# hyeeiin/ECG-Multimodal-Model

Hardware: AMD Instinct MI355X
Metric: samples/sec fwd+bwd, batch-256 multimodal (img+sig+clin), 1->8 MI355X (higher is better)
Workload: dtype bf16; 1 GPU; full multimodal (image 3x224x224 + 5000-pt signal + 16-dim clinical), fwd+bwd+Adam, encoders unfrozen; image_hw=224x224, per_gpu_batch=256, global_batch=256, parallelism=dp1

## Files before the change

ecg-multimodal-model_amd/csrc/api.hip:

```cpp
#include <stdarg.h>

#include "ops.h"

static thread_local char g_err[512] = "";

void ecg_set_error(const char* fmt, ...) {
  va_list ap;
  va_start(ap, fmt);
  vsnprintf(g_err, sizeof(g_err), fmt, ap);
  va_end(ap);
}

static inline ConvGeom geom_of(const ecgmm_conv_desc* c) {
  return make_geom(c->N, c->H, c->W, c->Cin, c->Cout, c->R, c->S, c->stride, c->pad_h, c->pad_w);
}
#define S_(x) ((hipStream_t)(x))

extern "C" {

int ecgmm_version(void) { return ECGMM_VERSION; }
const char* ecgmm_last_error(void) { return g_err; }

const char* ecgmm_switch_name(int i) { return i >= 0 && i < sw::COUNT ? sw::ALL[i]->env : nullptr; }
int ecgmm_switch_get(const char* env_name, int64_t* value) {
// ... 3 lines not shown
  *value = s->get();
  return 0;
}
int ecgmm_switch_set(const char* env_name, int64_t value) {
  Switch* s = sw::find(env_name);
  if (!s) ECG_FAIL(ECGMM_ERR_SHAPE, "switch_set: unknown switch %s", env_name ? env_name : "(null)");
  if (s == &sw::SIDE_WGRAD)
    ECG_FAIL(ECGMM_ERR_SHAPE, "switch_set: ECGMM_SIDE_WGRAD is each plan's own state after start-up, call ecgmm_side_wgrad()");
  if (!s->runtime) ECG_FAIL(ECGMM_ERR_SHAPE, "switch_set: %s is read once at start-up", s->env);
  s->set((long)value);
  return 0;
}
int ecgmm_conv_halo_enable(int on) { sw::CONV_HALO.set(on); return 0; }
int ecgmm_conv_halo_cus(int cus) { sw::HALO_CUS.set(cus); return 0; }
int ecgmm_conv_halo_w4(int on) { sw::HALO_W4.set(on); return 0; }
int ecgmm_conv_halo_stagger(int on) { sw::HALO_STAGGER.set(on); return 0; }
int ecgmm_conv_halo_stream(int on) { sw::HALO_STREAM.set(on); return 0; }
int ecgmm_conv_halo_pingpong(int on) { sw::HALO_PP.set(on); return 0; }
int ecgmm_conv_wgrad_pingpong(int on) { sw::WGRAD_PP.set(on); return 0; }
int ecgmm_conv_wgrad_ring_enable(int on) { sw::WGRAD_RING.set(on); return 0; }
int ecgmm_bn_fold(int on) { sw::BN_FOLD.set(on); return 0; }
int ecgmm_bn_fold_slice(int on) { sw::BN_FOLD_SLICE.set(on); return 0; }
int ecgmm_bn_dual(int on) { ecg_bn_dual_set(on); return 0; }
int ecgmm_bn_fuse_min_pixels(int64_t m) { sw::BN_FUSE_MIN_M.set((long)m); return 0; }
int ecgmm_stem_recompute(int on) { sw::STEM_RECOMPUTE.set(on); return 0; }
int ecgmm_infer_down_side(int on) { sw::INFER_DOWN_SIDE.set(on); return 0; }

int ecgmm_nchw_to_nhwc(int dtype, const float* src, void* dst, int N, int C, int64_t HW, void* stream) {
  return ecg_nchw_to_nhwc(dtype, src, dst, N, C, (long)HW, S_(stream));
}
int ecgmm_nhwc_to_nchw(int dtype, const void* src, float* dst, int N, int C, int64_t HW, void* stream) {
  return ecg_nhwc_to_nchw(dtype, src, dst, N, C, (long)HW, S_(stream));
}
int ecgmm_cast(int dtype, const float* src, void* dst, int64_t n, void* stream) {
  return ecg_cast(dtype, src, dst, (long)n, S_(stream));
}
int ecgmm_uncast(int dtype, const void* src, float* dst, int64_t n, void* stream) {
  return ecg_uncast(dtype, src, dst, (long)n, S_(stream));
}
int ecgmm_pack_conv_weight(int dtype, const float* w, void* fwd, void* dgrad, int Cout, int Cin, int RS,
                           void* stream) {
  return ecg_pack_weight(dtype, w, fwd, dgrad, Cout, Cin, RS, S_(stream));
}

int ecgmm_conv_stats_rows(int64_t out_pixels) { return ecg_conv_stats_rows((long)out_pixels); }
int ecgmm_conv_fwd(int dtype, const ecgmm_conv_desc* c, const void* x, const void* w_fwd, const float* bias, void* y,
// ... 28 lines not shown
}
int ecgmm_stem_stats_only_rows(int N, int Cin, int H, int W, int R) { return ecg_stem_stats_only_rows(N, Cin, H, W, R); }
int ecgmm_stem_stats_only(int dtype, const float* x, const void* packed, const float* bias, float* stats, int N, int Cin,
                          int H, int W, int R, void* stream) {
  return ecg_stem_stats_only(dtype, x, packed, bias, stats, N, Cin, H, W, R, S_(stream));
}
int ecgmm_stem_pool_fwd(const float* x, const void* packed, const float* coef, void* pooled, uint8_t* idx, int N, int Cin,
                        int H, int W, void* stream) {
  return ecg_stem_pool_fwd(x, packed, coef, pooled, idx, N, Cin, H, W, S_(stream));
}
size_t ecgmm_stem_pool_bwd_workspace(int N, int Cin, int H, int W) { return ecg_stem_pool_bwd_workspace(N, Cin, H, W); }
int ecgmm_stem_pool_bwd(const float* x, const void* packed, const float* coef, const float* gamma, const void* dp,
                        const void* pooled, const uint8_t* idx, float* dgamma, float* dbeta, float* dw_oihw, void* ws,
                        size_t ws_bytes, int N, int Cin, int H, int W, void* stream) {
  return ecg_stem_pool_bwd(x, packed, coef, gamma, dp, pooled, idx, dgamma, dbeta, dw_oihw, ws, ws_bytes, N, Cin, H, W,
                           S_(stream));
}
size_t ecgmm_stem_bwd_weight_workspace(int N, int Cin, int H, int W, int R) {
  return ecg_stem_wgrad_workspace(N, Cin, H, W, R);
}
int ecgmm_stem_bwd_weight(int dtype, const float* x, const void* dy, float* dw, int accumulate, void* ws,
                          size_t ws_bytes, int N, int Cin, int H, int W, int R, void* stream) {
  return ecg_stem_wgrad(dtype, x, dy, dw, accumulate, ws, ws_bytes, N, Cin, H, W, R, S_(stream));
}

int ecgmm_stem_bwd_data(int dtype, const void* dy, const float* w_oihw, float* dx, int N, int Cin, int H, int W, int R,
                        void* stream) {
  return ecg_stem_dgrad(dtype, dy, w_oihw, dx, N, Cin, H, W, R, S_(stream));
}

int ecgmm_bn_eval_bwd(int dtype, const void* dout, const void* maskref, const float* gate, const float* addc,
                      int rows_per_sample, const void* y, const float* coef, float* dgamma, float* dbeta, void* dy,
                      void* dz_out, float* dbias, int64_t M, int C, float* scratch, void* stream) {
  return ecg_bn_eval_bwd(dtype, dout, maskref, gate, addc, rows_per_sample, y, coef, dgamma, dbeta, dy, dz_out, dbias,
                         (long)M, C, scratch, S_(stream));
}
int ecgmm_bn_small_eval_bwd(const float* x, const float* dy, const float* gamma, const float* save, float* dx,
                            float* dgamma, float* dbeta, int N, int C, int accumulate, void* stream) {
  return ecg_bn_small_eval_bwd(x, dy, gamma, save, dx, dgamma, dbeta, N, C, accumulate, S_(stream));
}

int ecgmm_col_stats_rows(int dtype, int64_t M, int C) { return ecg_bn_rows(dtype, (long)M, C); }
int ecgmm_col_stats(int dtype, const void* x, int64_t M, int C, float* partial, void* stream) {
  int rows = 0;
  return ecg_col_stats(dtype, x, (long)M, C, partial, &rows, S_(stream));
}
// ... 298 lines not shown
```

ecg-multimodal-model_amd/csrc/conv_stem.hip:

```cpp
#include "ops.h"

__device__ __host__ inline size_t align_up_dev(size_t a) { return (a + 15) & ~(size_t)15; }

#ifndef STEM_ABL
#define STEM_ABL 0
#endif

namespace {

constexpr int STEM_CO = 64;
constexpr int MAXG = 24;

struct StemParams {
  const float* x;
  const void* wpk;
  void* y;
  const float* bias;
  float* stats;
  float* slab;
  int N, Cin, H, W, OH, OW, R, pad_h;
  int TH, TW;
  int tiles_h, tiles_w;
  int NG;
};
// ... 278 lines not shown
  }
#endif
  }
  __syncthreads();
  }
  if (STATS_WG && p.stats) {
    float* srow = p.stats + ((size_t)blockIdx.x * 4 + wave) * 2 * STEM_CO;
#pragma unroll
    for (int a = 0; a < 4; ++a) {
      f32x4 r1, r2;
#pragma unroll
      for (int j = 0; j < 4; ++j) {
        r1[j] = row16_sum(ws1[a][j]);
        r2[j] = row16_sum(ws2[a][j]);
      }
      if (fr == 0) {
        *reinterpret_cast<f32x4*>(srow + a * 16 + fq * 4) = r1;
        *reinterpret_cast<f32x4*>(srow + STEM_CO + a * 16 + fq * 4) = r2;
      }
    }
  }
}

template <typename T, int R>
__global__ __launch_bounds__(256) void stem_wgrad_kernel(StemParams p) {
  extern __shared__ __attribute__((aligned(16))) unsigned char smem[];
  constexpr int DYS = sizeof(T) == 2 ? 144 : 320;
  constexpr int TH = StemDims<R>::TH, TW = StemDims<R>::TW, PH = StemDims<R>::PH, PWS = StemDims<R>::PWS;
  unsigned char* sDY = smem;
  float* patch = reinterpret_cast<float*>(smem + 128 * DYS);

  const int tid = threadIdx.x, lane = tid & 63, wave = tid >> 6;
  const int fr = lane & 15, fq = lane >> 4;
  const int NK = p.NG * 8;
  const int ktiles = (NK + 15) / 16;
  const int tpi = p.tiles_h * p.tiles_w;
  const int vb = stem_xcd_order();
  const int pos = vb % tpi, slot = vb / tpi, nslots = gridDim.x / tpi;
  const int th_i = pos / p.tiles_w, tw_i = pos - th_i * p.tiles_w;
  const int oh0 = th_i * TH, ow0 = tw_i * TW;

  f32x4 acc[4][3];
#pragma unroll
  for (int a = 0; a < 4; ++a)
#pragma unroll
    for (int b = 0; b < 3; ++b) acc[a][b] = (f32x4){0.f, 0.f, 0.f, 0.f};

  int koff[3];
#pragma unroll
  for (int b = 0; b < 3; ++b) {
    const int kidx = (wave + 4 * b) * 16 + fr;
    const bool kok = (wave + 4 * b) < ktiles && kidx < NK;
    const int kk = kok ? kidx : 0;
    const int G = kk >> 3, c = G / R;
    koff[b] = (c * PH + (G - c * R)) * PWS + (kk & 7);
  }

  const T* dy = (const T*)p.y;
  constexpr int CH = 64 * (int)sizeof(T) / 16;
  constexpr int NDY = 128 * CH / 256;
  float pre[StemDims<R>::NPRE];
  u32x4 pdy[NDY];
  unsigned poff[StemDims<R>::NPRE], dyoff[NDY];
  stem_patch_offsets<R>(p, oh0, ow0, poff);
#pragma unroll
  for (int k = 0; k < NDY; ++k) {
    const int i = tid + 256 * k;
    const int pix = i / CH, chunk = i % CH;
    const int oh = oh0 + pix / TW, ow = ow0 + pix % TW;
    dyoff[k] = ((oh < p.OH) & (ow < p.OW)) ? (unsigned)(((oh * p.OW + ow) * STEM_CO) * (int)sizeof(T) + chunk * 16) : 0xFFFFFFFFu;
  }
  auto fetch = [&](int n) {
    const size_t dimg = (size_t)p.OH * p.OW * STEM_CO;
    const __amdgpu_buffer_rsrc_t drs = __builtin_amdgcn_make_buffer_rsrc((void*)(dy + (size_t)n * dimg), 0,
                                                                          (int)(dimg * sizeof(T)), 0x00020000);
#pragma unroll
    for (int k = 0; k < NDY; ++k) {
#if defined(__HIP_DEVICE_COMPILE__)
      pdy[k] = __builtin_amdgcn_raw_buffer_load_b128(drs, (int)dyoff[k], 0, 0);
#endif
    }
    stem_fetch_image_patch<R>(p, poff, pre, n);
  };
  if (slot < p.N) fetch(slot);
  for (int n = slot; n < p.N; n += nslots) {
    __syncthreads();
#pragma unroll
    for (int k = 0; k < NDY; ++k) {
      const int i = tid + 256 * k;
      *reinterpret_cast<u32x4*>(sDY + (i / CH) * DYS + (i % CH) * 16) = pdy[k];
    }
    stem_store_slots<float, R>(patch, pre);
    __syncthreads();
    if (n + nslots < p.N) fetch(n + nslots);

    if constexpr (sizeof(T) == 2) {
      const int q = fr >> 2, pq = fr & 3;
      for (int st = 0; st < 4; ++st) {
        u32x4 fa[4];
#pragma unroll
        for (int a = 0; a < 4; ++a) {
          const unsigned char* a0 = sDY + (st * 32 + 8 * fq + q) * DYS + (a * 16 + 4 * pq) * 2;
          s16x4 lo = __builtin_amdgcn_ds_read_tr16_b64_v4i16(
              (__attribute__((address_space(3))) s16x4*)(const_cast<unsigned char*>(a0)));
          s16x4 hi = __builtin_amdgcn_ds_read_tr16_b64_v4i16(
              (__attribute__((address_space(3))) s16x4*)(const_cast<unsigned char*>(a0 + 4 * DYS)));
          uint2 l2 = __builtin_bit_cast(uint2, lo), h2 = __builtin_bit_cast(uint2, hi);
          fa[a] = (u32x4){l2.x, l2.y, h2.x, h2.y};
        }
        const int pix0 = st * 32 + 8 * fq;
        const int trow = pix0 / TW, tcol0 = pix0 % TW;
#pragma unroll
        for (int b = 0; b < 3; ++b) {
          float bv[8];
          const float* src = patch + koff[b] + trow * 2 * PWS + tcol0 * 2;
#pragma unroll
          for (int j = 0; j < 8; ++j) bv[j] = src[2 * j];
          u32x4 fb = pack16<bf16_t>(bv);
#pragma unroll
          for (int a = 0; a < 4; ++a)
            mfma_bf16_inplace(acc[a][b], fa[a], fb);
        }
      }
    } else {
      for (int st = 0; st < 32; ++st) {
        const int pix = st * 4 + fq;
        const int trow = pix / TW, tcol = pix % TW;
        float fa[4];
#pragma unroll
        for (int a = 0; a < 4; ++a) fa[a] = *reinterpret_cast<const float*>(sDY + pix * DYS + (a * 16 + fr) * 4);
#pragma unroll
        for (int b = 0; b < 3; ++b) {
          float fb = patch[koff[b] + trow * 2 * PWS + tcol * 2];
#pragma unroll
          for (int a = 0; a < 4; ++a) acc[a][b] = __builtin_amdgcn_mfma_f32_16x16x4f32(fa[a], fb, acc[a][b], 0, 0, 0);
        }
      }
    }
  }

  if (sizeof(T) == 2) mfma_drain();
#pragma unroll
  for (int b = 0; b < 3; ++b) {
    int kidx = (wave + 4 * b) * 16 + fr;
    if ((wave + 4 * b) >= ktiles || kidx >= NK) continue;
#pragma unroll
    for (int a = 0; a < 4; ++a)
#pragma unroll
      for (int j = 0; j < 4; ++j)
        p.slab[((size_t)blockIdx.x * STEM_CO + a * 16 + fq * 4 + j) * NK + kidx] = acc[a][b][j];
  }
}

__global__ __launch_bounds__(256) void stem_wgrad_reduce_kernel(const float* __restrict__ slab,
                                                                float* __restrict__ grad, int nsplit, int NG,
                                                                int accumulate) {
  __shared__ float sh[16][17];
  const int oi = threadIdx.x & 15, sl = threadIdx.x >> 4;
  const int i = blockIdx.x * 16 + oi;
  const int total = STEM_CO * NG * 7;
  const int NK = NG * 8;
  float acc = 0.f;
  if (i < total) {
    int s = i % 7;
    int t = i / 7;
    int G = t % NG, co = t / NG;
    const float* src = slab + (size_t)co * NK + G * 8 + s;
    const size_t stride = (size_t)STEM_CO * NK;
    int k = sl;
    for (; k + 48 < nsplit; k += 64) {
      const float a0 = src[(size_t)k * stride], a1 = src[(size_t)(k + 16) * stride];
      const float a2 = src[(size_t)(k + 32) * stride], a3 = src[(size_t)(k + 48) * stride];
      acc += a0;
      acc += a1;
// ... 184 lines not shown
  if (!workspace || workspace_bytes < need)
    ECG_FAIL(ECGMM_ERR_WORKSPACE, "stem wgrad: workspace %zu < %zu", workspace_bytes, need);
  StemParams p;
  fill_params(p, s, N, Cin, H, W, R);
  p.x = x; p.y = const_cast<void*>(dy); p.slab = (float*)workspace;
  size_t lds = 128 * (size_t)(dtype == ECGMM_BF16 ? 144 : 320) + stem_patch_buffer_bytes(R, sizeof(float));
  if (dtype != ECGMM_BF16 && dtype != ECGMM_F32) ECG_FAIL(ECGMM_ERR_DTYPE, "stem wgrad: bad dtype %d", dtype);
  ecg_prof_begin(ECG_PROF_STEM_WGRAD, 2.0 * (double)N * s.OH * s.OW * STEM_CO * Cin * R * 7,
                 4.0 * N * Cin * H * W + (double)dtype_size(dtype) * N * s.OH * s.OW * STEM_CO, stream);
  if (dtype == ECGMM_BF16) {
    if (R == 7) hipLaunchKernelGGL((stem_wgrad_kernel<bf16_t, 7>), dim3(grid), dim3(256), lds, stream, p);
    else hipLaunchKernelGGL((stem_wgrad_kernel<bf16_t, 1>), dim3(grid), dim3(256), lds, stream, p);
  } else {
    if (R == 7) hipLaunchKernelGGL((stem_wgrad_kernel<float, 7>), dim3(grid), dim3(256), lds, stream, p);
    else hipLaunchKernelGGL((stem_wgrad_kernel<float, 1>), dim3(grid), dim3(256), lds, stream, p);
  }
  ecg_prof_end(stream);
  ECG_CHECK_LAUNCH("stem_wgrad");
  hipLaunchKernelGGL(stem_wgrad_reduce_kernel, dim3(ceil_div(STEM_CO * s.NG * 7, 16)), dim3(256), 0, stream,
                     (const float*)workspace, grad, grid, s.NG, accumulate);
  ECG_CHECK_LAUNCH("stem_wgrad_reduce");
  return 0;
}
```

ecg-multimodal-model_amd/csrc/ops.h:

```cpp
#pragma once
#include "common.h"
#include "switches.h"

int ecg_conv_stats_rows(long M);
struct ConvEpi {
  const void* red_y;
  const void* red_mask;
  const float* red_coef;
  float* red_rows;
  int wg_rows;
  const void* src2;
  const void* wpk2;
  int src2_done;
  int stats_rows;
  int red_done;
  int red_rows_n;
};
int ecg_conv_igemm(int dtype, int mode, const ConvGeom& g, const void* src, const void* wpk, void* dst,
                   const float* bias, const void* addend, float* stats, int act, hipStream_t stream,
                   ConvEpi* epi = nullptr);
bool ecg_conv_halo_ok(int dtype, int mode, const ConvGeom& g);
int ecg_conv_halo_rows(int mode, const ConvGeom& g);
int ecg_conv_halo(int mode, const ConvGeom& g, const void* src, const void* wpk, void* dst, const float* bias,
                  const void* addend, float* stats, int act, ConvEpi* epi, hipStream_t stream);
size_t ecg_conv_wgrad_workspace(int dtype, const ConvGeom& g);
void ecg_conv_wgrad_narrow(bool narrow, int slots = 256);
int ecg_conv_wgrad(int dtype, const ConvGeom& g, const void* x, const void* dy, float* grad_oihw, int accumulate,
                   void* workspace, size_t workspace_bytes, hipStream_t stream);
size_t ecg_stem_packed_elems(int Cin, int R);
int ecg_stem_stats_rows(int N, int Cin, int H, int W, int R);
int ecg_stem_pack(int dtype, const float* w, void* out, int Cin, int R, hipStream_t stream);
int ecg_stem_fwd(int dtype, const float* x, const void* wpk, const float* bias, void* y, float* stats, int N, int Cin,
                 int H, int W, int R, hipStream_t stream);
size_t ecg_stem_wgrad_workspace(int N, int Cin, int H, int W, int R);
int ecg_stem_wgrad(int dtype, const float* x, const void* dy, float* grad, int accumulate, void* workspace,
                   size_t workspace_bytes, int N, int Cin, int H, int W, int R, hipStream_t stream);
int ecg_stem_stats_only_rows(int N, int Cin, int H, int W, int R);
int ecg_stem_wg_stats_rows(int N, int Cin, int H, int W, int R);
int ecg_stem_fwd_wgrows(int dtype, const float* x, const void* wpk, const float* bias, void* y, float* stats, int N, int Cin,
                        int H, int W, int R, hipStream_t stream);
int ecg_stem_stats_only(int dtype, const float* x, const void* wpk, const float* bias, float* stats, int N, int Cin, int H,
                        int W, int R, hipStream_t stream);
int ecg_stem_wgrad_reduce(const float* slab, float* grad, int rows, int NG, int accumulate, hipStream_t stream);
int ecg_stem_dgrad(int dtype, const void* dy, const float* w, float* dx, int N, int Cin, int H, int W, int R,
                   hipStream_t stream);
bool ecg_stem_fused_ok(int dtype, int Cin, int R);
int ecg_stem_pool_fwd(const float* x, const void* wpk, const float* coef, void* pooled, unsigned char* idx, int N, int Cin,
                      int H, int W, hipStream_t stream);
size_t ecg_stem_pool_bwd_workspace(int N, int Cin, int H, int W);
int ecg_stem_pool_bwd(const float* x, const void* wpk, const float* coef, const float* gamma, const void* dp, const void* pooled,
                      const unsigned char* idx, float* dgamma, float* dbeta, float* dw, void* ws, size_t ws_bytes, int N,
                      int Cin, int H, int W, hipStream_t stream);
int ecg_pool_bn_bwd_reduce(int dtype, const void* dp, const void* pooled, const float* coef, const float* gamma, float* dgamma,
                           float* dbeta, int N, int H, int W, int C, float* scratch, const float** bcoef_out,
                           hipStream_t stream);
int ecg_bn_rows(int dtype, long M, int C);
int ecg_bn_finalize(const float* partial, int rows, int C, double count, const float* gamma, const float* beta,
                    float* rm, float* rv, long long* nbt, float momentum, float eps, float* coef, hipStream_t stream);
int ecg_bn_eval_coef(int C, const float* gamma, const float* beta, const float* rm, const float* rv, float eps,
                     float* coef, hipStream_t stream);
int ecg_col_stats(int dtype, const void* x, long M, int C, float* partial, int* rows_out, hipStream_t stream);
struct EcgBnFold {
  const float* partial; int rows; double count;
  const float* gamma; const float* beta;
  float* rm; float* rv; long long* nbt;
  float momentum, eps;
// ... 201 lines not shown
```

ecg-multimodal-model_amd/csrc/plan_resnet18.hip:

```cpp
#include "plan_common.h"
#include "side_stream.h"

namespace {
bool stem_recompute(int dtype) {
  return sw::STEM_RECOMPUTE.get() && ecg_stem_fused_ok(dtype, 3, 7);
}
bool relu_bits_on() { return sw::RELU_BITS.get() != 0; }

int build(const ecgmm_resnet18_desc* d, Net18& r) {
  ECG_TRY(net18_static(d, r, "resnet18"));
  return net18_shape(r, "resnet18");
}

struct FwdWs {
  void* wstem;
  void* y0; float* coef0; void* p0; unsigned char* idx0;
  BlockWs b[8];
  float* pooled;
  float* stats;
  float* stats_d;
  size_t bytes;
};

void layout_fwd(const Net18& r, void* base, FwdWs& w, WsTable* views = nullptr) {
// ... 375 lines not shown
        if (!sw::DOWN_FOLD.get()) ed.src2 = nullptr;
        if (ed.src2) {
          ECG_TRY(ecg_conv_igemm(dt, 1, g1, dy1b, b.w1d, din, nullptr, nullptr, nullptr, 0, s, &ed));
        }
        if (!ed.src2_done) {
          ECG_TRY(ecg_conv_igemm(dt, 1, gd, dydb, b.wdd, q.dtmp, nullptr, nullptr, nullptr, 0, s));
          ECG_TRY(ecg_conv_igemm(dt, 1, g1, dy1b, b.w1d, din, nullptr, q.dtmp, nullptr, 0, s));
        }
      } else {
        ConvEpi eb = {};
        if (fuse_here && i > 0 && ecg_conv_halo_ok(dt, 1, g1)) {
          const BlockWs& pb = w.b[i - 1];
          eb.wg_rows = 1; eb.red_y = pb.y2; eb.red_mask = pb.out; eb.red_coef = pb.coef2; eb.red_rows = q.red2;
        }
        ECG_TRY(ecg_conv_igemm(dt, 1, g1, dy1b, b.w1d, din, nullptr, dzp, nullptr, 0, s, &eb));
      }
    } else if (st == 9) {
      const void* dp0 = q.X[8 & 1];
      if (stem_recompute(dt)) {
        ECG_TRY(ecg_stem_pool_bwd(image, w.wstem, w.coef0, P(params, 1), dp0, w.p0, w.idx0, G(grads, 1), G(grads, 2),
                                  G(grads, 0), q.stem_ws, q.stem_bytes, N, 3, r.d.H, r.d.W, s));
        continue;
      }
      if (train && ecg_stem_fuse_on()) {
        ECG_TRY(ecg_pool_bn_bwd(dt, dp0, w.p0, w.idx0, w.y0, w.coef0, P(params, 1), G(grads, 1), G(grads, 2), q.big1,
                                nullptr, N, r.H1, r.W1, 64, q.bn_scratch, s));
      } else {
        ECG_TRY(ecg_maxpool_relu_bwd(dt, dp0, w.p0, w.idx0, q.big0, N, r.H1, r.W1, 64, s));
        ECG_TRY(bn_bwd_mode(r.bn, q.big0, nullptr, nullptr, nullptr, 1, w.y0, w.coef0, P(params, 1), G(grads, 1), G(grads, 2),
                            q.big1, nullptr, nullptr, (long)N * r.H1 * r.W1, 64, q.bn_scratch, s));
      }
      if (G(grads, 0)) {
        ECG_TRY(ecg_stem_wgrad(dt, image, q.big1, G(grads, 0), 0, q.stem_ws, q.stem_bytes, N, 3, r.d.H, r.d.W, 7, s));
      }
      if (dimage) ECG_TRY(ecg_stem_dgrad(dt, q.big1, P(params, 0), dimage, N, 3, r.d.H, r.d.W, 7, s));
    } else {
      ECG_FAIL(ECGMM_ERR_SHAPE, "resnet18 bwd: stage %d out of range", st);
    }
  }
  if (stage_end == 10) ecg_tl_mark(210, s);
  if (side && !g_side.defer_join) {
    hipEvent_t e = side_next_ev();
    (void)hipEventRecord(e, g_side.s);
    (void)hipStreamWaitEvent(s, e, 0);
  }
  if (stage_end == 10) ecg_tl_mark(211, s);
// ... 36 lines not shown
```

ecg-multimodal-model_amd/hip/lib.py:

```python
import ctypes as C
import os

F32, BF16 = 0, 1
ACT_NONE, ACT_RELU, ACT_SIGMOID = 0, 1, 2
RESNET18_NPARAMS, RESNET18_NBUFFERS = 62, 60
RESNET1D_NPARAMS, RESNET1D_NBUFFERS = 52, 27

_PKG_DIR = os.path.dirname(os.path.dirname(os.path.abspath(__file__)))
LIB_PATH = os.environ.get("ECGMM_LIB") or os.path.join(_PKG_DIR, "libecgmm_hip.so")

vp, i32, i64, u64, f32, f64, sz = C.c_void_p, C.c_int, C.c_int64, C.c_uint64, C.c_float, C.c_double, C.c_size_t


class ConvDesc(C.Structure):
    _fields_ = [(n, i32) for n in ("N", "H", "W", "Cin", "Cout", "R", "S", "stride", "pad_h", "pad_w")]


class ResNet18Desc(C.Structure):
    _fields_ = [("N", i32), ("H", i32), ("W", i32), ("out_dim", i32), ("dtype", i32), ("training", i32),
                ("bn_momentum", f32), ("bn_eps", f32)]


class ResNet1DDesc(C.Structure):
    _fields_ = [("N", i32), ("cin", i32), ("L", i32), ("num_classes", i32), ("dtype", i32), ("training", i32),
# ... 60 lines not shown
    "ecgmm_nhwc_to_nchw": (i32, [i32, vp, vp, i32, i32, i64, vp]),
    "ecgmm_cast": (i32, [i32, vp, vp, i64, vp]),
    "ecgmm_uncast": (i32, [i32, vp, vp, i64, vp]),
    "ecgmm_pack_conv_weight": (i32, [i32, vp, vp, vp, i32, i32, i32, vp]),
    "ecgmm_conv_stats_rows": (i32, [i64]),
    "ecgmm_conv_fwd": (i32, [i32, P(ConvDesc), vp, vp, vp, vp, vp, i32, vp]),
    "ecgmm_conv_fwd_wgrows": (i32, [i32, P(ConvDesc), vp, vp, vp, vp, vp, vp, i32, vp]),
    "ecgmm_conv_bwd_data": (i32, [i32, P(ConvDesc), vp, vp, vp, vp, vp]),
    "ecgmm_conv_bwd_weight_workspace": (sz, [i32, P(ConvDesc)]),
    "ecgmm_conv_bwd_weight": (i32, [i32, P(ConvDesc), vp, vp, vp, i32, vp, sz, vp]),
    "ecgmm_stem_packed_elems": (sz, [i32, i32]),
    "ecgmm_stem_stats_rows": (i32, [i32, i32, i32, i32, i32]),
    "ecgmm_stem_pack": (i32, [i32, vp, vp, i32, i32, vp]),
    "ecgmm_stem_fwd": (i32, [i32, vp, vp, vp, vp, vp, i32, i32, i32, i32, i32, vp]),
    "ecgmm_stem_wg_stats_rows": (i32, [i32, i32, i32, i32, i32]),
    "ecgmm_stem_fwd_wgrows": (i32, [i32, vp, vp, vp, vp, vp, i32, i32, i32, i32, i32, vp]),
    "ecgmm_stem_stats_only_rows": (i32, [i32, i32, i32, i32, i32]),
    "ecgmm_stem_stats_only": (i32, [i32, vp, vp, vp, vp, i32, i32, i32, i32, i32, vp]),
    "ecgmm_stem_pool_fwd": (i32, [vp, vp, vp, vp, vp, i32, i32, i32, i32, vp]),
    "ecgmm_stem_pool_bwd_workspace": (sz, [i32, i32, i32, i32]),
    "ecgmm_stem_pool_bwd": (i32, [vp, vp, vp, vp, vp, vp, vp, vp, vp, vp, vp, sz, i32, i32, i32, i32, vp]),
    "ecgmm_stem_bwd_weight_workspace": (sz, [i32, i32, i32, i32, i32]),
    "ecgmm_stem_bwd_weight": (i32, [i32, vp, vp, vp, i32, vp, sz, i32, i32, i32, i32, i32, vp]),
    "ecgmm_stem_bwd_data": (i32, [i32, vp, vp, vp, i32, i32, i32, i32, i32, vp]),
    "ecgmm_col_stats_rows": (i32, [i32, i64, i32]),
    "ecgmm_col_stats": (i32, [i32, vp, i64, i32, vp, vp]),
    "ecgmm_bn_finalize": (i32, [vp, i32, i32, f64, vp, vp, vp, vp, vp, f32, f32, vp, vp]),
    "ecgmm_bn_eval_coef": (i32, [i32, vp, vp, vp, vp, f32, vp, vp]),
    "ecgmm_bn_act": (i32, [i32, vp, vp, vp, vp, vp, i32, i32, vp, i64, i32, vp]),
    "ecgmm_bn_act_from_rows": (i32, [i32, vp, vp, i32, f64, vp, vp, vp, vp, vp, f32, f32, vp, vp, vp, vp, i32, i32, vp, i64, i32, vp]),
    "ecgmm_bn_bwd_scratch": (sz, [i32, i64, i32]),
    "ecgmm_bn_bwd": (i32, [i32, vp, vp, vp, vp, i32, vp, vp, vp, vp, vp, vp, vp, vp, i64, i32, vp, vp]),
    "ecgmm_bn_eval_bwd": (i32, [i32, vp, vp, vp, vp, i32, vp, vp, vp, vp, vp, vp, vp, i64, i32, vp, vp]),
    "ecgmm_conv_bwd_data_with_downsample": (i32, [i32, P(ConvDesc), vp, vp, vp, vp, vp, vp, vp]),
    "ecgmm_conv_bwd_data_bnred": (i32, [i32, P(ConvDesc), vp, vp, vp, vp, vp, vp, vp, vp, P(i32), vp]),
    "ecgmm_conv_bwd_data_bnred_rows": (i32, [i32, P(ConvDesc)]),
    "ecgmm_bn_bwd_from_rows": (i32, [i32, vp, vp, vp, vp, vp, vp, vp, vp, vp, i32, i64, i32, vp, vp]),
    "ecgmm_bnrelu_maxpool": (i32, [i32, vp, vp, vp, vp, i32, i32, i32, i32, vp]),
    "ecgmm_maxpool_relu_bwd": (i32, [i32, vp, vp, vp, vp, i32, i32, i32, i32, vp]),
    "ecgmm_bn_fuse_min_pixels": (i32, [i64]),
    "ecgmm_bn_fold": (i32, [i32]),
    "ecgmm_bn_fold_slice": (i32, [i32]),
    "ecgmm_bn_act_from_rows_bits": (i32, [i32, vp, vp, i32, f64, vp, vp, vp, vp, vp, f32, f32, vp, vp, vp, vp, i32, i32, vp, vp, i64, i32, vp]),
    "ecgmm_bn_bwd_bits": (i32, [i32, vp, vp, vp, vp, i32, vp, vp, vp, vp, vp, vp, vp, vp, i64, i32, vp, vp]),
    "ecgmm_bn_bwd_dual": (i32, [i32] + [vp] * 19 + [i64, i32, vp, vp, vp]),
    "ecgmm_bn_dual": (i32, [i32]),
# ... 101 lines not shown
LATER_SYMBOLS = ("ecgmm_resnet18_backward_dx", "ecgmm_resnet18_gradcam", "ecgmm_resnet1d_backward_dx",
                 "ecgmm_resnet1d_gradcam", "ecgmm_stem_bwd_data", "ecgmm_bn_eval_bwd", "ecgmm_bn_small_eval_bwd",
                 "ecgmm_resnet18_infer_prepared_bytes", "ecgmm_resnet18_infer_prepare", "ecgmm_resnet18_infer_workspace",
                 "ecgmm_resnet18_infer", "ecgmm_resnet1d_infer_prepared_bytes", "ecgmm_resnet1d_infer_prepare",
                 "ecgmm_resnet1d_infer_workspace", "ecgmm_resnet1d_infer", "ecgmm_infer_down_side", "ecgmm_conv_fwd_fused",
                 "ecgmm_fold_conv_bn", "ecgmm_relu_maxpool", "ecgmm_gate_res_relu",
                 "ecgmm_signal_filter_zscore", "ecgmm_signal_gather_augment",
                 "ecgmm_lstm_fwd_workspace", "ecgmm_lstm_bwd_workspace", "ecgmm_lstm_forward", "ecgmm_lstm_backward",
                 "ecgmm_conv5_in1_stats_rows", "ecgmm_conv5_in1_fwd", "ecgmm_conv5_in1_bwd_weight_workspace",
                 "ecgmm_conv5_in1_bwd_weight", "ecgmm_conv5_bwd_weight_workspace", "ecgmm_conv5_bwd_weight",
                 "ecgmm_bnrelu_maxpool2", "ecgmm_pool2_bn_bwd_workspace", "ecgmm_pool2_bn_bwd",
                 "ecgmm_crnn_front_fwd_workspace", "ecgmm_crnn_front_bwd_workspace", "ecgmm_crnn_front_forward",
                 "ecgmm_crnn_front_backward",
                 "ecgmm_switch_name", "ecgmm_switch_get", "ecgmm_switch_set",
                 "ecgmm_log_spectrogram_frames", "ecgmm_log_spectrogram",
                 "ecgmm_se_mlp_fwd", "ecgmm_se_mlp_bwd",
                 "ecgmm_signal_preprocess_i16", "ecgmm_weighted_sample",
                 "ecgmm_resnet18_ws_view", "ecgmm_resnet1d_ws_view",
                 "ecgmm_lime_perturb", "ecgmm_lime_ridge_workspace", "ecgmm_lime_ridge", "ecgmm_lime_prob",
                 "ecgmm_shap_mlp_workspace", "ecgmm_shap_gradient", "ecgmm_shap_deep",
                 "ecgmm_bn_bwd_dual", "ecgmm_bn_dual",
                 "ecgmm_mha_bwd_workspace", "ecgmm_mha_forward", "ecgmm_mha_backward", "ecgmm_mha_keep_mask",
                 "ecgmm_embed1d_fwd", "ecgmm_embed1d_bwd_workspace", "ecgmm_embed1d_bwd",
                 "ecgmm_se_gate_bn")

_lib = None


def _missing(name):
    def fail(*_a):
        raise RuntimeError(f"{LIB_PATH} does not export {name}: rebuild the HIP library (there is no fallback)")
    return fail


def lib():
    global _lib
    if _lib is None:
        if not os.path.exists(LIB_PATH):
            raise RuntimeError(
                f"libecgmm_hip.so not found at {LIB_PATH}: the HIP extension is the only compute path "
                "(no CPU fallback). Build it with `python __graft_entry__.py` or "
                "`make -C ecg-multimodal-model_amd/csrc`.")
        import torch
        h = C.CDLL(LIB_PATH)
        for name, (res, args) in SIGNATURES.items():
            if name in LATER_SYMBOLS and os.environ.get("ECGMM_LIB") and not hasattr(h, name):
                setattr(h, name, _missing(name))
# ... 14 lines not shown
```

include/ecgmm.h:

```cpp
#ifndef ECGMM_H
#define ECGMM_H
#include <stddef.h>
#include <stdint.h>

#ifdef __cplusplus
extern "C" {
#endif

#define ECGMM_VERSION 100

enum { ECGMM_F32 = 0, ECGMM_BF16 = 1 };
enum { ECGMM_ACT_NONE = 0, ECGMM_ACT_RELU = 1, ECGMM_ACT_SIGMOID = 2 };
enum {
  ECGMM_OK = 0,
  ECGMM_ERR_SHAPE = 1,
  ECGMM_ERR_DTYPE = 2,
  ECGMM_ERR_WORKSPACE = 3,
  ECGMM_ERR_LAUNCH = 4
};

int ecgmm_version(void);
const char* ecgmm_last_error(void);

const char* ecgmm_switch_name(int i);
// ... 113 lines not shown
int ecgmm_conv_wgrad_pingpong(int on);
int ecgmm_conv_wgrad_ring_enable(int on);
int ecgmm_conv_fwd(int dtype, const ecgmm_conv_desc* c, const void* x, const void* w_fwd, const float* bias, void* y,
                   float* stats, int act, void* stream);
int ecgmm_conv_fwd_wgrows(int dtype, const ecgmm_conv_desc* c, const void* x, const void* w_fwd, const float* bias, void* y,
                          float* stats, int* nrows, int act, void* stream);
int ecgmm_conv_bwd_data(int dtype, const ecgmm_conv_desc* c, const void* dy, const void* w_dgrad, const void* addend,
                        void* dx, void* stream);
size_t ecgmm_conv_bwd_weight_workspace(int dtype, const ecgmm_conv_desc* c);
int ecgmm_conv_bwd_weight(int dtype, const ecgmm_conv_desc* c, const void* x, const void* dy, float* dw_oihw,
                          int accumulate, void* ws, size_t ws_bytes, void* stream);

size_t ecgmm_stem_packed_elems(int Cin, int R);
int ecgmm_stem_stats_rows(int N, int Cin, int H, int W, int R);
int ecgmm_stem_pack(int dtype, const float* w_oihw, void* packed, int Cin, int R, void* stream);
int ecgmm_stem_fwd(int dtype, const float* x, const void* packed, const float* bias, void* y, float* stats, int N,
                   int Cin, int H, int W, int R, void* stream);
int ecgmm_stem_wg_stats_rows(int N, int Cin, int H, int W, int R);
int ecgmm_stem_fwd_wgrows(int dtype, const float* x, const void* packed, const float* bias, void* y, float* stats, int N,
                          int Cin, int H, int W, int R, void* stream);
size_t ecgmm_stem_bwd_weight_workspace(int N, int Cin, int H, int W, int R);
int ecgmm_stem_bwd_weight(int dtype, const float* x, const void* dy, float* dw_oihw, int accumulate, void* ws,
                          size_t ws_bytes, int N, int Cin, int H, int W, int R, void* stream);
int ecgmm_stem_bwd_data(int dtype, const void* dy, const float* w_oihw, float* dx, int N, int Cin, int H, int W, int R,
                        void* stream);

int ecgmm_stem_stats_only_rows(int N, int Cin, int H, int W, int R);
int ecgmm_stem_stats_only(int dtype, const float* x, const void* packed, const float* bias, float* stats, int N, int Cin,
                          int H, int W, int R, void* stream);
int ecgmm_stem_pool_fwd(const float* x, const void* packed, const float* coef, void* pooled, uint8_t* idx, int N, int Cin,
                        int H, int W, void* stream);
size_t ecgmm_stem_pool_bwd_workspace(int N, int Cin, int H, int W);
int ecgmm_stem_pool_bwd(const float* x, const void* packed, const float* coef, const float* gamma, const void* dp,
                        const void* pooled, const uint8_t* idx, float* dgamma, float* dbeta, float* dw_oihw, void* ws,
                        size_t ws_bytes, int N, int Cin, int H, int W, void* stream);

#define ECGMM_BN_TAIL_ROWS 64
int ecgmm_col_stats_rows(int dtype, int64_t M, int C);
int ecgmm_col_stats(int dtype, const void* x, int64_t M, int C, float* partial, void* stream);
int ecgmm_bn_finalize(const float* partial, int rows, int C, double count, const float* gamma, const float* beta,
                      float* running_mean, float* running_var, int64_t* num_batches_tracked, float momentum, float eps,
                      float* coef, void* stream);
int ecgmm_bn_eval_coef(int C, const float* gamma, const float* beta, const float* running_mean,
                       const float* running_var, float eps, float* coef, void* stream);
int ecgmm_bn_act(int dtype, const void* y, const float* coef, const void* res, const float* rcoef, const float* gate,
                 int rows_per_sample, int relu, void* out, int64_t M, int C, void* stream);
// ... 17 lines not shown
                                        const void* dy_down, const void* w_down_dgrad, void* dx, void* tmp,
                                        void* stream);
int ecgmm_bn_bwd_from_rows(int dtype, const void* dout, const void* maskref, const void* y, const float* coef,
                           const float* gamma, float* dgamma, float* dbeta, void* dy, const float* rows, int nrows,
                           int64_t M, int C, void* scratch, void* stream);

int ecgmm_bn_fuse_min_pixels(int64_t m);
int ecgmm_bn_fold(int on);
int ecgmm_bn_fold_slice(int on);
int ecgmm_bn_act_from_rows_bits(int dtype, const void* y, const float* partial, int rows, double count, const float* gamma,
                                const float* beta, float* running_mean, float* running_var, int64_t* num_batches_tracked,
                                float momentum, float eps, float* coef_out, const void* res, const float* rcoef,
                                const float* gate, int rows_per_sample, int relu, void* out, uint8_t* relu_bits, int64_t M,
                                int C, void* stream);
int ecgmm_bn_bwd_bits(int dtype, const void* dout, const uint8_t* mask_bits, const float* gate, const float* addc,
                      int rows_per_sample, const void* y, const float* coef, const float* gamma, float* dgamma,
                      float* dbeta, void* dy, void* dz_out, float* dbias, int64_t M, int C, void* scratch, void* stream);
int ecgmm_bn_bwd_dual(int dtype, const void* dout, const void* maskref, const uint8_t* mask_bits, const float* gate,
                      const float* addc, const void* y_a, const float* coef_a, const float* gamma_a, float* dgamma_a,
                      float* dbeta_a, void* dy_a, const void* y_b, const float* coef_b, const float* gamma_b,
                      float* dgamma_b, float* dbeta_b, void* dy_b, void* dz, float* dbias, int64_t M, int C, void* scratch_a,
                      void* scratch_b, void* stream);
int ecgmm_bn_dual(int on);
int ecgmm_stem_recompute(int on);

int ecgmm_bnrelu_maxpool(int dtype, const void* y, const float* coef, void* out, uint8_t* idx, int N, int H, int W,
                         int C, void* stream);
int ecgmm_maxpool_relu_bwd(int dtype, const void* dp, const void* pooled, const uint8_t* idx, void* dz, int N, int H,
                           int W, int C, void* stream);
int ecgmm_pool_bn_bwd(int dtype, const void* dp, const void* pooled, const uint8_t* idx, const void* y, const float* coef,
                      const float* gamma, float* dgamma, float* dbeta, void* dy, float* dbias, int N, int H, int W, int C,
                      void* scratch, void* stream);
int ecgmm_avgpool(int dtype, const void* x, float* out, int N, int R, int C, const float* coef, void* stream);
int ecgmm_bcast_rows(int dtype, const float* v, void* out, int N, int R, int C, float scale, void* stream);
int ecgmm_se_gate_grad(int dtype, const void* dout, const void* maskref, const void* y, const float* coef, float* dg,
                       int N, int R, int C, void* stream);
int ecgmm_se_gate_bn(int dtype, const void* dout, const void* maskref, const void* y, const float* coef, void* dz, float* dg,
                     float* a1, float* a2, float* a3, int N, int R, int C, void* stream);
int ecgmm_se_mlp_fwd(const float* m, const float* w1, const float* b1, const float* w2, const float* b2, float* h, float* g,
                     int N, int C, int CR, void* stream);
int ecgmm_se_mlp_bwd(const float* dg, const float* g, const float* h, const float* m, const float* w1, const float* w2,
                     float* ds, float* dh, float* dm, float* dw1, float* db1, float* dw2, float* db2, int N, int C, int CR,
                     float scale, void* stream);

int ecgmm_linear_fwd(const float* x, const float* w, const float* bias, float* y, int B, int In, int Out, int act,
                     void* stream);
// ... 170 lines not shown
```

Before: 40540 samples/s.

## Fuse stem maxpool/BN backward elementwise pass into the stem weight-gradient kernel

Adds a fused stem backward kernel that rebuilds the BN-input gradient on the fly from the pooled gradient, pooled values, argmax indices and pre-BN activations, writes it straight into LDS, and feeds it to the existing MFMA weight-gradient tile loop. A separate reduce pass still computes the BN gradient coefficients first. This removes writing the full-resolution dy tensor to global memory and reading it back in the wgrad kernel. The cost is extra loads and ALU work per tile, plus higher register pressure in the wgrad kernel. The path is on by default for bf16 training when the image gradient is not needed.

```diff
diff --git a/ecg-multimodal-model_amd/csrc/api.hip b/ecg-multimodal-model_amd/csrc/api.hip
--- a/ecg-multimodal-model_amd/csrc/api.hip
+++ b/ecg-multimodal-model_amd/csrc/api.hip
@@ -49,6 +49,7 @@
 int ecgmm_bn_fold(int on) { sw::BN_FOLD.set(on); return 0; }
 int ecgmm_bn_fold_slice(int on) { sw::BN_FOLD_SLICE.set(on); return 0; }
 int ecgmm_bn_dual(int on) { ecg_bn_dual_set(on); return 0; }
+int ecgmm_stem_bwd_fuse(int on) { ecg_stem_bwd_fused_set(on); return 0; }
 int ecgmm_bn_fuse_min_pixels(int64_t m) { sw::BN_FUSE_MIN_M.set((long)m); return 0; }
 int ecgmm_stem_recompute(int on) { sw::STEM_RECOMPUTE.set(on); return 0; }
 int ecgmm_infer_down_side(int on) { sw::INFER_DOWN_SIDE.set(on); return 0; }
@@ -123,6 +124,12 @@
 int ecgmm_stem_bwd_weight(int dtype, const float* x, const void* dy, float* dw, int accumulate, void* ws,
                           size_t ws_bytes, int N, int Cin, int H, int W, int R, void* stream) {
   return ecg_stem_wgrad(dtype, x, dy, dw, accumulate, ws, ws_bytes, N, Cin, H, W, R, S_(stream));
+}
+int ecgmm_stem_bwd_fused(int dtype, const float* x, const void* dp, const void* pooled, const uint8_t* idx, const void* y,
+                         const float* coef, const float* gamma, float* dgamma, float* dbeta, float* dw, int accumulate,
+                         void* scratch, void* ws, size_t ws_bytes, int N, int Cin, int H, int W, void* stream) {
+  return ecg_stem_bwd_fused(dtype, x, dp, pooled, idx, y, coef, gamma, dgamma, dbeta, dw, accumulate, (float*)scratch, ws,
+                            ws_bytes, N, Cin, H, W, S_(stream));
 }
 
 int ecgmm_stem_bwd_data(int dtype, const void* dy, const float* w_oihw, float* dx, int N, int Cin, int H, int W, int R,
diff --git a/ecg-multimodal-model_amd/csrc/conv_stem.hip b/ecg-multimodal-model_amd/csrc/conv_stem.hip
--- a/ecg-multimodal-model_amd/csrc/conv_stem.hip
+++ b/ecg-multimodal-model_amd/csrc/conv_stem.hip
@@ -324,6 +324,64 @@
   }
 }
 
+template <int R>
+__device__ __forceinline__ void stem_wgrad_koff(int wave, int fr, int ktiles, int NK, int (&koff)[3]) {
+  constexpr int PH = StemDims<R>::PH, PWS = StemDims<R>::PWS;
+#pragma unroll
+  for (int b = 0; b < 3; ++b) {
+    const int kidx = (wave + 4 * b) * 16 + fr;
+    const bool kok = (wave + 4 * b) < ktiles && kidx < NK;
+    const int kk = kok ? kidx : 0;
+    const int G = kk >> 3, c = G / R;
+    koff[b] = (c * PH + (G - c * R)) * PWS + (kk & 7);
+  }
+}
+template <int R, int DYS>
+__device__ __forceinline__ void stem_wgrad_tile_bf16(const unsigned char* sDY, const float* patch, const int (&koff)[3], int fr,
+                                                     int fq, f32x4 (&acc)[4][3]) {
+  constexpr int TW = StemDims<R>::TW, PWS = StemDims<R>::PWS;
+  const int q = fr >> 2, pq = fr & 3;
+  for (int st = 0; st < 4; ++st) {
+    u32x4 fa[4];
+#pragma unroll
+    for (int a = 0; a < 4; ++a) {
+      const unsigned char* a0 = sDY + (st * 32 + 8 * fq + q) * DYS + (a * 16 + 4 * pq) * 2;
+      s16x4 lo = __builtin_amdgcn_ds_read_tr16_b64_v4i16(
+          (__attribute__((address_space(3))) s16x4*)(const_cast<unsigned char*>(a0)));
+      s16x4 hi = __builtin_amdgcn_ds_read_tr16_b64_v4i16(
+          (__attribute__((address_space(3))) s16x4*)(const_cast<unsigned char*>(a0 + 4 * DYS)));
+      uint2 l2 = __builtin_bit_cast(uint2, lo), h2 = __builtin_bit_cast(uint2, hi);
+      fa[a] = (u32x4){l2.x, l2.y, h2.x, h2.y};
+    }
+    const int pix0 = st * 32 + 8 * fq;
+    const int trow = pix0 / TW, tcol0 = pix0 % TW;
+#pragma unroll
+    for (int b = 0; b < 3; ++b) {
+      float bv[8];
+      const float* src = patch + koff[b] + trow * 2 * PWS + tcol0 * 2;
+#pragma unroll
+      for (int j = 0; j < 8; ++j) bv[j] = src[2 * j];
+      u32x4 fb = pack16<bf16_t>(bv);
+#pragma unroll
+      for (int a = 0; a < 4; ++a)
+        mfma_bf16_inplace(acc[a][b], fa[a], fb);
+    }
+  }
+}
+__device__ __forceinline__ void stem_wgrad_store_slab(float* slab, const f32x4 (&acc)[4][3], int wave, int fr, int fq, int ktiles,
+                                                      int NK) {
+#pragma unroll
+  for (int b = 0; b < 3; ++b) {
+    int kidx = (wave + 4 * b) * 16 + fr;
+    if ((wave + 4 * b) >= ktiles || kidx >= NK) continue;
+#pragma unroll
+    for (int a = 0; a < 4; ++a)
+#pragma unroll
+      for (int j = 0; j < 4; ++j)
+        slab[((size_t)blockIdx.x * STEM_CO + a * 16 + fq * 4 + j) * NK + kidx] = acc[a][b][j];
+  }
+}
+
 template <typename T, int R>
 __global__ __launch_bounds__(256) void stem_wgrad_kernel(StemParams p) {
   extern __shared__ __attribute__((aligned(16))) unsigned char smem[];
@@ -349,14 +407,7 @@
     for (int b = 0; b < 3; ++b) acc[a][b] = (f32x4){0.f, 0.f, 0.f, 0.f};
 
   int koff[3];
-#pragma unroll
-  for (int b = 0; b < 3; ++b) {
-    const int kidx = (wave + 4 * b) * 16 + fr;
-    const bool kok = (wave + 4 * b) < ktiles && kidx < NK;
-    const int kk = kok ? kidx : 0;
-    const int G = kk >> 3, c = G / R;
-    koff[b] = (c * PH + (G - c * R)) * PWS + (kk & 7);
-  }
+  stem_wgrad_koff<R>(wave, fr, ktiles, NK, koff);
 
   const T* dy = (const T*)p.y;
   constexpr int CH = 64 * (int)sizeof(T) / 16;
@@ -397,33 +448,7 @@
     if (n + nslots < p.N) fetch(n + nslots);
 
     if constexpr (sizeof(T) == 2) {
-      const int q = fr >> 2, pq = fr & 3;
-      for (int st = 0; st < 4; ++st) {
-        u32x4 fa[4];
-#pragma unroll
-        for (int a = 0; a < 4; ++a) {
-          const unsigned char* a0 = sDY + (st * 32 + 8 * fq + q) * DYS + (a * 16 + 4 * pq) * 2;
-          s16x4 lo = __builtin_amdgcn_ds_read_tr16_b64_v4i16(
-              (__attribute__((address_space(3))) s16x4*)(const_cast<unsigned char*>(a0)));
-          s16x4 hi = __builtin_amdgcn_ds_read_tr16_b64_v4i16(
-              (__attribute__((address_space(3))) s16x4*)(const_cast<unsigned char*>(a0 + 4 * DYS)));
-          uint2 l2 = __builtin_bit_cast(uint2, lo), h2 = __builtin_bit_cast(uint2, hi);
-          fa[a] = (u32x4){l2.x, l2.y, h2.x, h2.y};
-        }
-        const int pix0 = st * 32 + 8 * fq;
-        const int trow = pix0 / TW, tcol0 = pix0 % TW;
-#pragma unroll
-        for (int b = 0; b < 3; ++b) {
-          float bv[8];
-          const float* src = patch + koff[b] + trow * 2 * PWS + tcol0 * 2;
-#pragma unroll
-          for (int j = 0; j < 8; ++j) bv[j] = src[2 * j];
-          u32x4 fb = pack16<bf16_t>(bv);
-#pragma unroll
-          for (int a = 0; a < 4; ++a)
-            mfma_bf16_inplace(acc[a][b], fa[a], fb);
-        }
-      }
+      stem_wgrad_tile_bf16<R, DYS>(sDY, patch, koff, fr, fq, acc);
     } else {
       for (int st = 0; st < 32; ++st) {
         const int pix = st * 4 + fq;
@@ -442,16 +467,161 @@
   }
 
   if (sizeof(T) == 2) mfma_drain();
-#pragma unroll
-  for (int b = 0; b < 3; ++b) {
-    int kidx = (wave + 4 * b) * 16 + fr;
-    if ((wave + 4 * b) >= ktiles || kidx >= NK) continue;
-#pragma unroll
-    for (int a = 0; a < 4; ++a)
-#pragma unroll
-      for (int j = 0; j < 4; ++j)
-        p.slab[((size_t)blockIdx.x * STEM_CO + a * 16 + fq * 4 + j) * NK + kidx] = acc[a][b][j];
-  }
+  stem_wgrad_store_slab(p.slab, acc, wave, fr, fq, ktiles, NK);
+}
+
+struct StemBwdParams {
+  StemParams s;
+  const bf16_t* dp;
+  const bf16_t* pooled;
+  const unsigned char* idx;
+  const float* coef;
+  const float* bcoef;
+  int QH, QW;
+};
+
+__global__ __launch_bounds__(256) void stem_bwd_fused_kernel(StemBwdParams q) {
+  using T = bf16_t;
+  constexpr int R = 7, C = STEM_CO, VEC = 8;
+  const StemParams& p = q.s;
+  extern __shared__ __attribute__((aligned(16))) unsigned char smem[];
+  constexpr int DYS = 144;
+  constexpr int TH = StemDims<R>::TH, TW = StemDims<R>::TW;
+  unsigned char* sDY = smem;
+  float* patch = reinterpret_cast<float*>(smem + 128 * DYS);
+  float* sK = patch + StemDims<R>::NPRE * 256;
+
+  const int tid = threadIdx.x, lane = tid & 63, wave = tid >> 6;
+  const int fr = lane & 15, fq = lane >> 4;
+  const int NK = p.NG * 8;
+  const int ktiles = (NK + 15) / 16;
+  const int tpi = p.tiles_h * p.tiles_w;
+  const int vb = stem_xcd_order();
+  const int pos = vb % tpi, slot = vb / tpi, nslots = gridDim.x / tpi;
+  const int th_i = pos / p.tiles_w, tw_i = pos - th_i * p.tiles_w;
+  const int oh0 = th_i * TH, ow0 = tw_i * TW;
+
+  f32x4 acc[4][3];
+#pragma unroll
+  for (int a = 0; a < 4; ++a)
+#pragma unroll
+    for (int b = 0; b < 3; ++b) acc[a][b] = (f32x4){0.f, 0.f, 0.f, 0.f};
+
+  int koff[3];
+  stem_wgrad_koff<R>(wave, fr, ktiles, NK, koff);
+
+  if (tid < C) {
+    const float mean = q.coef[2 * C + tid], inv = q.coef[3 * C + tid];
+    const float k1 = q.bcoef[tid];
+    const float bn = -k1 * q.bcoef[2 * C + tid] * inv;
+    const float an = -k1 * q.bcoef[C + tid] - bn * mean;
+    sK[tid] = k1;
+    sK[C + tid] = bn;
+    sK[2 * C + tid] = an;
+  }
+
+  const int chunk = tid & 7, bc = (tid >> 3) & 7, br = tid >> 6;
+  const int c0 = chunk * VEC;
+  const int h0 = oh0 + 2 * br, w0 = ow0 + 2 * bc;
+  const int k = h0 >> 1, m = w0 >> 1;
+  const bool inb = h0 < p.OH && w0 < p.OW;
+  const bool okw = inb && w0 + 1 < p.OW, okh = inb && h0 + 1 < p.OH;
+  bool wok[4];
+  unsigned woff[4], yoff[4];
+#pragma unroll
+  for (int a = 0; a < 2; ++a)
+#pragma unroll
+    for (int b = 0; b < 2; ++b) {
+      const int w = a * 2 + b;
+      wok[w] = inb && k + a < q.QH && m + b < q.QW;
+      woff[w] = wok[w] ? (unsigned)((((k + a) * q.QW + m + b) * C + c0) * 2) : 0xFFFFFFFFu;
+      const bool pok = a ? (b ? okh && okw : okh) : (b ? okw : inb);
+      yoff[w] = pok ? (unsigned)((((h0 + a) * p.OW + w0 + b) * C + c0) * 2) : 0xFFFFFFFFu;
+    }
+  const bool pixok[4] = {inb, okw, okh, okh && okw};
+
+  float pre[StemDims<R>::NPRE];
+  unsigned poff[StemDims<R>::NPRE];
+  stem_patch_offsets<R>(p, oh0, ow0, poff);
+  u32x4 rd[4], rp[4], ry[4];
+  uint2 pk[4];
+  const size_t qimg = (size_t)q.QH * q.QW * C, yimg = (size_t)p.OH * p.OW * C;
+  auto fetch = [&](int n) {
+#if defined(__HIP_DEVICE_COMPILE__)
+    const __amdgpu_buffer_rsrc_t r_dp = __builtin_amdgcn_make_buffer_rsrc((void*)(q.dp + (size_t)n * qimg), 0, (int)(qimg * 2), 0x00020000);
+    const __amdgpu_buffer_rsrc_t r_pp = __builtin_amdgcn_make_buffer_rsrc((void*)(q.pooled + (size_t)n * qimg), 0, (int)(qimg * 2), 0x00020000);
+    const __amdgpu_buffer_rsrc_t r_ix = __builtin_amdgcn_make_buffer_rsrc((void*)(q.idx + (size_t)n * qimg), 0, (int)qimg, 0x00020000);
+    const __amdgpu_buffer_rsrc_t r_y = __builtin_amdgcn_make_buffer_rsrc((void*)((const T*)p.y + (size_t)n * yimg), 0, (int)(yimg * 2), 0x00020000);
+#pragma unroll
+    for (int w = 0; w < 4; ++w) {
+      rd[w] = __builtin_amdgcn_raw_buffer_load_b128(r_dp, (int)woff[w], 0, 0);
+      rp[w] = __builtin_amdgcn_raw_buffer_load_b128(r_pp, (int)woff[w], 0, 0);
+      const auto t2 = __builtin_amdgcn_raw_buffer_load_b64(r_ix, (int)(woff[w] >> 1), 0, 0);
+      pk[w] = make_uint2(t2[0], t2[1]);
+    }
+#pragma unroll
+    for (int px = 0; px < 4; ++px) ry[px] = __builtin_amdgcn_raw_buffer_load_b128(r_y, (int)yoff[px], 0, 0);
+#endif
+    stem_fetch_image_patch<R>(p, poff, pre, n);
+  };
+  if (slot < p.N) fetch(slot);
+  __syncthreads();
+  for (int n = slot; n < p.N; n += nslots) {
+    u32x4 orow[4];
+    {
+      float k1[VEC], bn[VEC], an[VEC];
+#pragma unroll
+      for (int j = 0; j < VEC; j += 4) {
+        *reinterpret_cast<float4*>(k1 + j) = *reinterpret_cast<const float4*>(sK + c0 + j);
+        *reinterpret_cast<float4*>(bn + j) = *reinterpret_cast<const float4*>(sK + C + c0 + j);
+        *reinterpret_cast<float4*>(an + j) = *reinterpret_cast<const float4*>(sK + 2 * C + c0 + j);
+      }
+      float d[4][VEC];
+#pragma unroll
+      for (int w = 0; w < 4; ++w) {
+        float pv[VEC];
+        unpack16<T>(rd[w], d[w]);
+        unpack16<T>(rp[w], pv);
+#pragma unroll
+        for (int j = 0; j < VEC; ++j) d[w][j] = (wok[w] && pv[j] > 0.f) ? d[w][j] : 0.f;
+      }
+      auto g = [&](int w, int tap, int j) -> float {
+        const unsigned word = (j >> 2) ? pk[w].y : pk[w].x;
+        const int code = (int)((word >> (8 * (j & 3))) & 0xffu);
+        return code == tap ? d[w][j] : 0.f;
+      };
+#pragma unroll
+      for (int px = 0; px < 4; ++px) {
+        float v[VEC], o[VEC];
+        unpack16<T>(ry[px], v);
+#pragma unroll
+        for (int j = 0; j < VEC; ++j) {
+          float z;
+          if (px == 0) z = g(0, 4, j);
+          else if (px == 1) z = g(0, 5, j) + g(1, 3, j);
+          else if (px == 2) z = g(0, 7, j) + g(2, 1, j);
+          else z = ((g(0, 8, j) + g(1, 6, j)) + g(2, 2, j)) + g(3, 0, j);
+          o[j] = k1[j] * z + (bn[j] * v[j] + an[j]);
+        }
+        const u32x4 r = pack16<T>(o);
+        orow[px] = pixok[px] ? r : (u32x4){0u, 0u, 0u, 0u};
+      }
+    }
+    __syncthreads();
+#pragma unroll
+    for (int px = 0; px < 4; ++px) {
+      const int pix = (2 * br + (px >> 1)) * TW + 2 * bc + (px & 1);
+      *reinterpret_cast<u32x4*>(sDY + pix * DYS + chunk * 16) = orow[px];
+    }
+    stem_store_slots<float, R>(patch, pre);
+    __syncthreads();
+    if (n + nslots < p.N) fetch(n + nslots);
+
+    stem_wgrad_tile_bf16<R, DYS>(sDY, patch, koff, fr, fq, acc);
+  }
+
+  mfma_drain();
+  stem_wgrad_store_slab(p.slab, acc, wave, fr, fq, ktiles, NK);
 }
 
 __global__ __launch_bounds__(256) void stem_wgrad_reduce_kernel(const float* __restrict__ slab,
@@ -682,3 +852,41 @@
   ECG_CHECK_LAUNCH("stem_wgrad_reduce");
   return 0;
 }
+
+static int g_stem_bwd_fused = 1;
+void ecg_stem_bwd_fused_set(int on) { g_stem_bwd_fused = on != 0; }
+bool ecg_stem_bwd_fused_on() { return g_stem_bwd_fused != 0; }
+bool ecg_stem_bwd_fused_ok(int dtype, int Cin) { return dtype == ECGMM_BF16 && Cin >= 1 && Cin <= 3; }
+
+int ecg_stem_bwd_fused(int dtype, const float* x, const void* dp, const void* pooled, const unsigned char* idx, const void* y,
+                       const float* coef, const float* gamma, float* dgamma, float* dbeta, float* grad, int accumulate,
+                       float* scratch, void* workspace, size_t workspace_bytes, int N, int Cin, int H, int W,
+                       hipStream_t stream) {
+  constexpr int R = 7;
+  if (!ecg_stem_bwd_fused_ok(dtype, Cin))
+    ECG_FAIL(ECGMM_ERR_DTYPE, "stem bwd fused: bf16 and Cin <= 3 only (dtype %d, Cin %d)", dtype, Cin);
+  StemShape s;
+  ECG_TRY(stem_shape(Cin, H, W, R, s));
+  const int grid = stem_wgrad_grid(N, s.tiles_h * s.tiles_w);
+  size_t need = (size_t)grid * STEM_CO * s.NG * 8 * sizeof(float);
+  if (!workspace || workspace_bytes < need)
+    ECG_FAIL(ECGMM_ERR_WORKSPACE, "stem bwd fused: workspace %zu < %zu", workspace_bytes, need);
+  if (!x || !dp || !pooled || !idx || !y || !coef || !scratch || !grad) ECG_FAIL(ECGMM_ERR_SHAPE, "stem bwd fused: null operand");
+  StemBwdParams q;
+  memset(&q, 0, sizeof(q));
+  fill_params(q.s, s, N, Cin, H, W, R);
+  q.s.x = x; q.s.y = const_cast<void*>(y); q.s.slab = (float*)workspace;
+  q.dp = (const bf16_t*)dp; q.pooled = (const bf16_t*)pooled; q.idx = idx; q.coef = coef;
+  q.QH = (s.OH - 1) / 2 + 1; q.QW = (s.OW - 1) / 2 + 1;
+  ECG_TRY(ecg_pool_bn_bwd_reduce(dtype, dp, pooled, coef, gamma, dgamma, dbeta, N, s.OH, s.OW, STEM_CO, scratch, &q.bcoef, stream));
+  const size_t lds = 128 * (size_t)144 + stem_patch_buffer_bytes(R, sizeof(float)) + 3 * STEM_CO * sizeof(float);
+  const double px = (double)N * s.OH * s.OW * STEM_CO;
+  ecg_prof_begin(ECG_PROF_STEM_WGRAD, 2.0 * px * Cin * R * 7, 4.0 * N * Cin * H * W + 2.0 * px + 5.0 * N * q.QH * q.QW * STEM_CO, stream);
+  hipLaunchKernelGGL(stem_bwd_fused_kernel, dim3(grid), dim3(256), lds, stream, q);
+  ecg_prof_end(stream);
+  ECG_CHECK_LAUNCH("stem_bwd_fused");
+  hipLaunchKernelGGL(stem_wgrad_reduce_kernel, dim3(ceil_div(STEM_CO * s.NG * 7, 16)), dim3(256), 0, stream,
+                     (const float*)workspace, grad, grid, s.NG, accumulate);
+  ECG_CHECK_LAUNCH("stem_wgrad_reduce");
+  return 0;
+}
diff --git a/ecg-multimodal-model_amd/csrc/ops.h b/ecg-multimodal-model_amd/csrc/ops.h
--- a/ecg-multimodal-model_amd/csrc/ops.h
+++ b/ecg-multimodal-model_amd/csrc/ops.h
@@ -42,6 +42,13 @@
 int ecg_stem_stats_only(int dtype, const float* x, const void* wpk, const float* bias, float* stats, int N, int Cin, int H,
                         int W, int R, hipStream_t stream);
 int ecg_stem_wgrad_reduce(const float* slab, float* grad, int rows, int NG, int accumulate, hipStream_t stream);
+bool ecg_stem_bwd_fused_ok(int dtype, int Cin);
+void ecg_stem_bwd_fused_set(int on);
+bool ecg_stem_bwd_fused_on();
+int ecg_stem_bwd_fused(int dtype, const float* x, const void* dp, const void* pooled, const unsigned char* idx, const void* y,
+                       const float* coef, const float* gamma, float* dgamma, float* dbeta, float* grad, int accumulate,
+                       float* scratch, void* workspace, size_t workspace_bytes, int N, int Cin, int H, int W,
+                       hipStream_t stream);
 int ecg_stem_dgrad(int dtype, const void* dy, const float* w, float* dx, int N, int Cin, int H, int W, int R,
                    hipStream_t stream);
 bool ecg_stem_fused_ok(int dtype, int Cin, int R);
diff --git a/ecg-multimodal-model_amd/csrc/plan_resnet18.hip b/ecg-multimodal-model_amd/csrc/plan_resnet18.hip
--- a/ecg-multimodal-model_amd/csrc/plan_resnet18.hip
+++ b/ecg-multimodal-model_amd/csrc/plan_resnet18.hip
@@ -421,6 +421,11 @@
                                   G(grads, 0), q.stem_ws, q.stem_bytes, N, 3, r.d.H, r.d.W, s));
         continue;
       }
+      if (train && ecg_stem_fuse_on() && ecg_stem_bwd_fused_on() && ecg_stem_bwd_fused_ok(dt, 3) && !dimage && G(grads, 0)) {
+        ECG_TRY(ecg_stem_bwd_fused(dt, image, dp0, w.p0, w.idx0, w.y0, w.coef0, P(params, 1), G(grads, 1), G(grads, 2),
+                                   G(grads, 0), 0, q.bn_scratch, q.stem_ws, q.stem_bytes, N, 3, r.d.H, r.d.W, s));
+        continue;
+      }
       if (train && ecg_stem_fuse_on()) {
         ECG_TRY(ecg_pool_bn_bwd(dt, dp0, w.p0, w.idx0, w.y0, w.coef0, P(params, 1), G(grads, 1), G(grads, 2), q.big1,
                                 nullptr, N, r.H1, r.W1, 64, q.bn_scratch, s));
diff --git a/ecg-multimodal-model_amd/hip/lib.py b/ecg-multimodal-model_amd/hip/lib.py
--- a/ecg-multimodal-model_amd/hip/lib.py
+++ b/ecg-multimodal-model_amd/hip/lib.py
@@ -106,6 +106,8 @@
     "ecgmm_stem_pool_bwd": (i32, [vp, vp, vp, vp, vp, vp, vp, vp, vp, vp, vp, sz, i32, i32, i32, i32, vp]),
     "ecgmm_stem_bwd_weight_workspace": (sz, [i32, i32, i32, i32, i32]),
     "ecgmm_stem_bwd_weight": (i32, [i32, vp, vp, vp, i32, vp, sz, i32, i32, i32, i32, i32, vp]),
+    "ecgmm_stem_bwd_fused": (i32, [i32, vp, vp, vp, vp, vp, vp, vp, vp, vp, vp, i32, vp, vp, sz, i32, i32, i32, i32, vp]),
+    "ecgmm_stem_bwd_fuse": (i32, [i32]),
     "ecgmm_stem_bwd_data": (i32, [i32, vp, vp, vp, i32, i32, i32, i32, i32, vp]),
     "ecgmm_col_stats_rows": (i32, [i32, i64, i32]),
     "ecgmm_col_stats": (i32, [i32, vp, i64, i32, vp, vp]),
@@ -253,7 +255,8 @@
                  "ecgmm_bn_bwd_dual", "ecgmm_bn_dual",
                  "ecgmm_mha_bwd_workspace", "ecgmm_mha_forward", "ecgmm_mha_backward", "ecgmm_mha_keep_mask",
                  "ecgmm_embed1d_fwd", "ecgmm_embed1d_bwd_workspace", "ecgmm_embed1d_bwd",
-                 "ecgmm_se_gate_bn")
+                 "ecgmm_se_gate_bn",
+                 "ecgmm_stem_bwd_fused", "ecgmm_stem_bwd_fuse")
 
 _lib = None
 
diff --git a/include/ecgmm.h b/include/ecgmm.h
--- a/include/ecgmm.h
+++ b/include/ecgmm.h
@@ -159,6 +159,9 @@
 size_t ecgmm_stem_bwd_weight_workspace(int N, int Cin, int H, int W, int R);
 int ecgmm_stem_bwd_weight(int dtype, const float* x, const void* dy, float* dw_oihw, int accumulate, void* ws,
                           size_t ws_bytes, int N, int Cin, int H, int W, int R, void* stream);
+int ecgmm_stem_bwd_fused(int dtype, const float* x, const void* dp, const void* pooled, const uint8_t* idx, const void* y,
+                         const float* coef, const float* gamma, float* dgamma, float* dbeta, float* dw_oihw, int accumulate,
+                         void* scratch, void* ws, size_t ws_bytes, int N, int Cin, int H, int W, void* stream);
 int ecgmm_stem_bwd_data(int dtype, const void* dy, const float* w_oihw, float* dx, int N, int Cin, int H, int W, int R,
                         void* stream);
 
@@ -222,6 +225,7 @@
                       float* dgamma_b, float* dbeta_b, void* dy_b, void* dz, float* dbias, int64_t M, int C, void* scratch_a,
                       void* scratch_b, void* stream);
 int ecgmm_bn_dual(int on);
+int ecgmm_stem_bwd_fuse(int on);
 int ecgmm_stem_recompute(int on);
 
 int ecgmm_bnrelu_maxpool(int dtype, const void* y, const float* coef, void* out, uint8_t* idx, int N, int H, int W,
```

After: 40830 samples/s, median of 6. No clear change (+0.7%).
